# SitaoLuan/When-Do-GNNs-Help

Measured on AMD Instinct MI355X. Metric: aggregation edges/sec (whole job; + %HBM roofline of the SpMM kernel), higher is better.
Workload: dtype f32; 1 GPU; synthetic homophily sweep (data_synthesis/4000-equivalent): 10 h-levels x 5 seeds = 50 graphs/GPU/step, N=2000 nodes, k=10, F=500 fp32, C=5; step = batched D^-1(A+I)X aggregation + edge/label stati...; parallelism=independent sweep shards x1 (no data-path collective; job-table broadcast + r...

## Files before the change

when-do-gnns-help_amd/csrc/spmm_narrow.hip:

```cpp
#include <algorithm>

#include "wdg_common.h"

namespace {
using namespace wdg;

constexpr int N_THREADS = 256;
constexpr int N_WAVES = N_THREADS / kWave;

typedef unsigned short bf16_t;

template <typename TIN>
__device__ __forceinline__ float n_f32(TIN v);
template <>
__device__ __forceinline__ float n_f32<float>(float v) { return v; }
template <>
__device__ __forceinline__ float n_f32<bf16_t>(bf16_t v) { return __uint_as_float(static_cast<unsigned>(v) << 16); }

template <typename TIN>
__global__ __launch_bounds__(256) void narrow_pack(const TIN *__restrict__ X, int64_t ldx, const float *__restrict__ cs, int n_cols,
                                                   int F, float *__restrict__ T) {
    const int64_t i = static_cast<int64_t>(blockIdx.x) * 256 + threadIdx.x;
    if (i >= static_cast<int64_t>(n_cols) * 8) return;
    const int c = static_cast<int>(i >> 3), f = static_cast<int>(i & 7);
    float v = 0.f;
    if (f < F) v = n_f32<TIN>(X[static_cast<int64_t>(c) * ldx + f]) * (cs ? cs[c] : 1.f);
    T[i] = v;
}

template <typename TIN>
__global__ __launch_bounds__(256) void narrow_pack4(const TIN *__restrict__ X, int64_t ldx, const float *__restrict__ cs, int n_cols,
                                                    int F, float *__restrict__ T) {
    const int64_t i = static_cast<int64_t>(blockIdx.x) * 256 + threadIdx.x;
    if (i >= static_cast<int64_t>(n_cols) * 4) return;
    const int c = static_cast<int>(i >> 2), f = static_cast<int>(i & 3);
    float v = 0.f;
    if (f < F) v = n_f32<TIN>(X[static_cast<int64_t>(c) * ldx + f]) * (cs ? cs[c] : 1.f);
    T[i] = v;
}
__global__ __launch_bounds__(256) void narrow_pack_bf16x8(const bf16_t *__restrict__ X, int64_t ldx, int n_cols, int F,
                                                          bf16_t *__restrict__ T) {
    const int64_t i = static_cast<int64_t>(blockIdx.x) * 256 + threadIdx.x;
    if (i >= static_cast<int64_t>(n_cols) * 8) return;
    const int c = static_cast<int>(i >> 3), f = static_cast<int>(i & 7);
    T[i] = f < F ? X[static_cast<int64_t>(c) * ldx + f] : static_cast<bf16_t>(0);
}

enum { TABLE_F32X8 = 0, TABLE_F32X4 = 1, TABLE_BF16X8 = 2 };

struct Acc8 {
    float v[8];
};

__device__ __forceinline__ void narrow_unpack_bf16(const f32x4_t raw, f32x4_t &lo, f32x4_t &hi) {
    const unsigned w0 = __float_as_uint(raw[0]), w1 = __float_as_uint(raw[1]), w2 = __float_as_uint(raw[2]), w3 = __float_as_uint(raw[3]);
    lo[0] = __uint_as_float(w0 << 16); lo[1] = __uint_as_float(w0 & 0xffff0000u);
    lo[2] = __uint_as_float(w1 << 16); lo[3] = __uint_as_float(w1 & 0xffff0000u);
    hi[0] = __uint_as_float(w2 << 16); hi[1] = __uint_as_float(w2 & 0xffff0000u);
    hi[2] = __uint_as_float(w3 << 16); hi[3] = __uint_as_float(w3 & 0xffff0000u);
}

template <int G, bool HAS_W, bool WIDE = true, bool BF16 = false>
__device__ __forceinline__ Acc8 narrow_sweep(global_ptr<const int32_t> col, global_ptr<const float> val,
                                             global_ptr<const f32x4_t> T, int b, int e, int sub, int64_t ldq = 2,
                                             global_ptr<const float> cs = nullptr) {
    Acc8 a;
#pragma unroll
    for (int f = 0; f < 8; ++f) a.v[f] = 0.f;
    const f32x4_t zero = {0.f, 0.f, 0.f, 0.f};
    int k = b + sub;
    for (; k + 3 * G < e; k += 4 * G) {
        int idx[4];
        float w[4];
        f32x4_t lo[4], hi[4];
#pragma unroll
        for (int u = 0; u < 4; ++u) idx[u] = col[k + u * G];
#pragma unroll
        for (int u = 0; u < 4; ++u) {
            lo[u] = T[ldq * static_cast<int64_t>(idx[u])];
            hi[u] = (WIDE && !BF16) ? T[ldq * static_cast<int64_t>(idx[u]) + 1] : zero;
            w[u] = 1.f;
            if (HAS_W) w[u] = (val ? val[k + u * G] : 1.f) * (cs ? cs[idx[u]] : 1.f);
        }
#pragma unroll
        for (int u = 0; u < 4; ++u) {
            if (BF16) narrow_unpack_bf16(lo[u], lo[u], hi[u]);
#pragma unroll
            for (int f = 0; f < 4; ++f) {
                a.v[f] = HAS_W ? __builtin_fmaf(w[u], lo[u][f], a.v[f]) : a.v[f] + lo[u][f];
                if (WIDE) a.v[4 + f] = HAS_W ? __builtin_fmaf(w[u], hi[u][f], a.v[4 + f]) : a.v[4 + f] + hi[u][f];
            }
        }
    }
    for (; k < e; k += G) {
        const int idx = col[k];
        f32x4_t lo = T[ldq * static_cast<int64_t>(idx)], hi = (WIDE && !BF16) ? T[ldq * static_cast<int64_t>(idx) + 1] : zero;
        if (BF16) narrow_unpack_bf16(lo, lo, hi);
        float w = 1.f;
        if (HAS_W) w = (val ? val[k] : 1.f) * (cs ? cs[idx] : 1.f);
#pragma unroll
        for (int f = 0; f < 4; ++f) {
            a.v[f] = HAS_W ? __builtin_fmaf(w, lo[f], a.v[f]) : a.v[f] + lo[f];
            if (WIDE) a.v[4 + f] = HAS_W ? __builtin_fmaf(w, hi[f], a.v[4 + f]) : a.v[4 + f] + hi[f];
        }
    }
    return a;
}

__device__ __forceinline__ float narrow_reduce16(const Acc8 &a, int lane) {
    float h4[4], h2[2];
    const bool b3 = lane & 8, b2 = lane & 4, b1 = lane & 2;
#pragma unroll
    for (int i = 0; i < 4; ++i) {
        const float keep = b3 ? a.v[4 + i] : a.v[i], send = b3 ? a.v[i] : a.v[4 + i];
        h4[i] = keep + __shfl_xor(send, 8);
    }
#pragma unroll
    for (int i = 0; i < 2; ++i) {
        const float keep = b2 ? h4[2 + i] : h4[i], send = b2 ? h4[i] : h4[2 + i];
        h2[i] = keep + __shfl_xor(send, 4);
    }
    const float keep = b1 ? h2[1] : h2[0], send = b1 ? h2[0] : h2[1];
    const float h1 = keep + __shfl_xor(send, 2);
    return h1 + __shfl_xor(h1, 1);
}

__device__ __forceinline__ float narrow_reduce64(Acc8 a, int lane) {
#pragma unroll
    for (int f = 0; f < 8; ++f) a.v[f] += __shfl_xor(a.v[f], 32);
#pragma unroll
    for (int f = 0; f < 8; ++f) a.v[f] += __shfl_xor(a.v[f], 16);
    return narrow_reduce16(a, lane);
}

template <bool HAS_VAL, int TABLE = TABLE_F32X8>
__global__ __launch_bounds__(N_THREADS) void spmm_narrow_kernel(const wdg_spmm_job job, const float *__restrict__ Tf,
                                                                const int32_t *__restrict__ part_ptr, int parts,
                                                                float *__restrict__ P) {
    __shared__ float part_sums[N_WAVES][8];
    constexpr bool WIDE = TABLE != TABLE_F32X4, BF16 = TABLE == TABLE_BF16X8;
    constexpr int64_t LDQ = TABLE == TABLE_F32X8 ? 2 : 1;
    const global_ptr<const int32_t> rowptr = to_global(job.rowptr), col = to_global(job.col), perm = to_global(job.band_perm);
    const global_ptr<const int32_t> pptr = to_global(part_ptr);
    const global_ptr<const float> val = to_global(job.val), rs = to_global(job.row_scale);
    const global_ptr<const f32x4_t> T = (global_ptr<const f32x4_t>)Tf;
    const int N = job.n_rows, F = job.n_feat;
    const int n_wg_rows = job.band_cuts[18], n_wave_rows = job.band_cuts[19];
    const int tid = threadIdx.x, wave = tid >> 6, lane = tid & 63;
    const int feat = (lane >> 1) & 7;
    const int xcd = blockIdx.x % kXcds, per_part = kXcds / parts;
    const int part = xcd / per_part;
    const int wg = (xcd % per_part) + per_part * (blockIdx.x / kXcds), n_wgs = gridDim.x / parts;
    const bool direct = parts == 1;
    const global_ptr<float> out = direct ? to_global(job.Y) : to_global(P) + static_cast<int64_t>(part) * N * 8;
    const int64_t ldo = direct ? job.ldy : 8;
    const int n_out = direct ? F : 8;
    auto bounds = [&](int row, int &b, int &e) {
        b = rowptr[row], e = rowptr[row + 1];
        if (!direct) {
            const global_ptr<const int32_t> pp = pptr + static_cast<int64_t>(row) * (parts - 1);
            if (part > 0) b = pp[part - 1];
            if (part + 1 < parts) e = pp[part];
        }
    };
    auto scale_of = [&](int row) { return (direct && rs) ? rs[row] : 1.f; };

    for (int i = wg; i < n_wg_rows; i += n_wgs) {
        const int row = perm[i];
        int b, e;
        bounds(row, b, e);
        const float total = narrow_reduce64(narrow_sweep<N_THREADS, HAS_VAL, WIDE, BF16>(col, val, T, b, e, tid, LDQ), lane);
        if (lane < 16 && !(lane & 1)) part_sums[wave][feat] = total;
        __syncthreads();
        if (tid < n_out) {
            float sum = part_sums[0][tid];
#pragma unroll
            for (int w = 1; w < N_WAVES; ++w) sum += part_sums[w][tid];
            out[static_cast<int64_t>(row) * ldo + tid] = sum * scale_of(row);
        }
        __syncthreads();
    }
    const int gwave = wg * N_WAVES + wave, n_gwaves = n_wgs * N_WAVES;
    for (int i = n_wg_rows + gwave; i < n_wave_rows; i += n_gwaves) {
        const int row = perm[i];
        int b, e;
        bounds(row, b, e);
        const float total = narrow_reduce64(narrow_sweep<kWave, HAS_VAL, WIDE, BF16>(col, val, T, b, e, lane, LDQ), lane);
        if (lane < 16 && !(lane & 1) && feat < n_out) out[static_cast<int64_t>(row) * ldo + feat] = total * scale_of(row);
    }
    const int rest = N - n_wave_rows;
    for (int q = gwave; q * 4 < rest; q += n_gwaves) {
        const int slot = q * 4 + (lane >> 4);
        const bool live = slot < rest;
        const int row = live ? perm[n_wave_rows + slot] : 0;
        int b = 0, e = 0;
        if (live) bounds(row, b, e);
        const float total = narrow_reduce16(narrow_sweep<16, HAS_VAL, WIDE, BF16>(col, val, T, b, e, lane & 15, LDQ), lane);
        if (live && !(lane & 1) && feat < n_out) out[static_cast<int64_t>(row) * ldo + feat] = total * scale_of(row);
    }
}

__global__ __launch_bounds__(256) void narrow_plan_kernel(const int32_t *__restrict__ rowptr, const int32_t *__restrict__ col, int N,
                                                          int part_cols, int parts, int32_t *__restrict__ part_ptr) {
    const int64_t i = static_cast<int64_t>(blockIdx.x) * 256 + threadIdx.x;
    if (i >= static_cast<int64_t>(N) * (parts - 1)) return;
    const int row = static_cast<int>(i / (parts - 1)), p = static_cast<int>(i % (parts - 1)) + 1;
    int lo = rowptr[row], hi = rowptr[row + 1];
    const int key = p * part_cols;
    while (lo < hi) {
        const int mid = (lo + hi) >> 1;
        if (col[mid] < key) lo = mid + 1;
        else hi = mid;
    }
    part_ptr[i] = lo;
}

__global__ __launch_bounds__(256) void narrow_combine(const float *__restrict__ P, int N, int parts, int F, const float *__restrict__ rs,
                                                      float *__restrict__ Y, int64_t ldy) {
    const int64_t i = static_cast<int64_t>(blockIdx.x) * 256 + threadIdx.x;
    if (i >= static_cast<int64_t>(N) * 8) return;
    const int row = static_cast<int>(i >> 3), f = static_cast<int>(i & 7);
    if (f >= F) return;
    float sum = P[i];
    for (int p = 1; p < parts; ++p) sum += P[static_cast<int64_t>(p) * N * 8 + i];
    Y[static_cast<int64_t>(row) * ldy + f] = sum * (rs ? rs[row] : 1.f);
}

template <bool HAS_W, bool WIDE>
__global__ __launch_bounds__(N_THREADS) void spmm_narrow_batched_kernel(const wdg_spmm_job *__restrict__ jobs, int blocks_per_job) {
    const int job_id = blockIdx.x / blocks_per_job, rb = blockIdx.x % blocks_per_job;
    const desc_ptr<wdg_spmm_job> job = (desc_ptr<wdg_spmm_job>)(jobs + job_id);
    const int N = job->n_rows, F = job->n_feat;
    const int lane = threadIdx.x & 63;
    const int row = rb * 16 + (threadIdx.x >> 4);
    if (rb * 16 >= N) return;
    const global_ptr<const int32_t> rowptr = to_global(job->rowptr), col = to_global(job->col);
    const global_ptr<const float> val = to_global(job->val), rs = to_global(job->row_scale), cs = to_global(job->col_scale);
    const global_ptr<const f32x4_t> X = (global_ptr<const f32x4_t>)to_global(static_cast<const float *>(job->X));
    const bool live = row < N;
    const int b = live ? rowptr[row] : 0, e = live ? rowptr[row + 1] : 0;
    const float total = narrow_reduce16(narrow_sweep<16, HAS_W, WIDE>(col, val, X, b, e, lane & 15, job->ldx / 4, cs), lane);
    const int feat = (lane >> 1) & 7;
    if (live && !(lane & 1) && feat < F) to_global(job->Y)[static_cast<int64_t>(row) * job->ldy + feat] = total * (rs ? rs[row] : 1.f);
}

constexpr int64_t N_PART_BYTES = 3 << 20;

}

extern "C" {

int32_t wdg_spmm_narrow_col_bytes(int32_t n_feat, int32_t x_is_bf16, int32_t has_col_scale) {
    return (n_feat <= 4 || (x_is_bf16 && !has_col_scale)) ? 16 : 32;
}

int32_t wdg_spmm_narrow_parts(int32_t n_cols, int32_t col_bytes) {
    if (const char *s = getenv("WDG_NARROW_PARTS")) {
        const int v = atoi(s);
        if (v == 1 || v == 2 || v == 4 || v == 8) return v;
    }
    int parts = 1;
    while (parts < 8 && static_cast<int64_t>(n_cols) * col_bytes > N_PART_BYTES * parts) parts <<= 1;
    return parts;
}

size_t wdg_spmm_narrow_workspace_bytes(int32_t n_rows, int32_t n_cols) {
    const int parts = wdg_spmm_narrow_parts(n_cols, 32);
    return static_cast<size_t>(n_cols > 0 ? n_cols : 0) * 32 + (parts > 1 ? static_cast<size_t>(parts) * (n_rows > 0 ? n_rows : 0) * 32 : 0) + 512;
}

int wdg_spmm_narrow_plan(const int32_t *rowptr, const int32_t *col, int32_t N, int32_t n_cols, int32_t parts, int32_t *part_ptr,
                         wdg_stream_t stream) {
    WDG_REQUIRE(N >= 0 && n_cols >= 0, "spmm_narrow_plan: negative size");
    WDG_REQUIRE(parts == 1 || parts == 2 || parts == 4 || parts == 8, "spmm_narrow_plan: parts must be 1, 2, 4 or 8");
    if (parts == 1 || N == 0) return WDG_OK;
    WDG_REQUIRE(rowptr && col && part_ptr, "spmm_narrow_plan: null array");
    const int part_cols = static_cast<int>(wdg::ceil_div(n_cols, parts));
    const int64_t threads = static_cast<int64_t>(N) * (parts - 1);
    hipLaunchKernelGGL(narrow_plan_kernel, dim3(static_cast<unsigned>(wdg::ceil_div(threads, 256))), dim3(256), 0, wdg::as_stream(stream),
                       rowptr, col, N, part_cols, parts, part_ptr);
    return wdg::check_launch("narrow_plan_kernel");
}

static int narrow_launch(const wdg_spmm_job *j, bool bf16, const int32_t *part_ptr, void *workspace, size_t workspace_bytes,
                         wdg_stream_t stream) {
    WDG_REQUIRE(j != nullptr, "spmm_narrow: null job");
    WDG_REQUIRE(j->n_rows >= 0 && j->n_cols >= 0 && j->n_feat >= 0, "spmm_narrow: negative size");
    if (j->n_rows == 0 || j->n_feat == 0) return WDG_OK;
    if (j->n_feat > 8) return wdg::fail(WDG_ERR_UNSUPPORTED, "spmm_narrow: more than 8 features (use wdg_spmm_csr_*)");
    WDG_REQUIRE(j->rowptr && j->Y && (j->n_cols == 0 || j->X), "spmm_narrow: null rowptr / X / Y");
    WDG_REQUIRE(j->band_perm && j->band_cuts, "spmm_narrow: the job carries no band plan (wdg_csr_band_plan)");
    WDG_REQUIRE(j->ldx >= j->n_feat && j->ldy >= j->n_feat, "spmm_narrow: leading dimension smaller than n_feat");
    WDG_REQUIRE(j->y_group_stride == 0, "spmm_narrow: Y must be row-major (y_group_stride is the quad-row kernel's)");
    const int col_bytes = wdg_spmm_narrow_col_bytes(j->n_feat, bf16 ? 1 : 0, j->col_scale ? 1 : 0);
    const int table = col_bytes == 32 ? TABLE_F32X8 : (j->n_feat <= 4 ? TABLE_F32X4 : TABLE_BF16X8);
    const int parts = wdg_spmm_narrow_parts(j->n_cols, col_bytes);
    WDG_REQUIRE(parts == 1 || part_ptr, "spmm_narrow: this column count needs the split positions of wdg_spmm_narrow_plan");
    if (!workspace || workspace_bytes < wdg_spmm_narrow_workspace_bytes(j->n_rows, j->n_cols))
        return wdg::fail(WDG_ERR_WORKSPACE, "spmm_narrow: workspace too small");
    hipStream_t st = wdg::as_stream(stream);
    float *T = reinterpret_cast<float *>((reinterpret_cast<uintptr_t>(workspace) + 255) & ~static_cast<uintptr_t>(255));
    float *P = T + static_cast<size_t>(j->n_cols) * 8;
    if (j->n_cols > 0) {
        const int per_col = table == TABLE_F32X4 ? 4 : 8;
        const unsigned blocks = static_cast<unsigned>(wdg::ceil_div(static_cast<int64_t>(j->n_cols) * per_col, 256));
        if (table == TABLE_BF16X8)
            hipLaunchKernelGGL(narrow_pack_bf16x8, dim3(blocks), dim3(256), 0, st, static_cast<const bf16_t *>(j->X), j->ldx, j->n_cols, j->n_feat, reinterpret_cast<bf16_t *>(T));
        else if (table == TABLE_F32X4 && bf16)
            hipLaunchKernelGGL(narrow_pack4<bf16_t>, dim3(blocks), dim3(256), 0, st, static_cast<const bf16_t *>(j->X), j->ldx, j->col_scale, j->n_cols, j->n_feat, T);
        else if (table == TABLE_F32X4)
            hipLaunchKernelGGL(narrow_pack4<float>, dim3(blocks), dim3(256), 0, st, static_cast<const float *>(j->X), j->ldx, j->col_scale, j->n_cols, j->n_feat, T);
        else if (bf16)
            hipLaunchKernelGGL(narrow_pack<bf16_t>, dim3(blocks), dim3(256), 0, st, static_cast<const bf16_t *>(j->X), j->ldx, j->col_scale, j->n_cols, j->n_feat, T);
        else
            hipLaunchKernelGGL(narrow_pack<float>, dim3(blocks), dim3(256), 0, st, static_cast<const float *>(j->X), j->ldx, j->col_scale, j->n_cols, j->n_feat, T);
    }
    const int cus = std::max(wdg_device_cus(), 8);
    const int per_cu = 8;
    const dim3 grid(static_cast<unsigned>(cus / kXcds * kXcds * per_cu));
#define WDG_NARROW_LAUNCH(V, TB) hipLaunchKernelGGL((spmm_narrow_kernel<V, TB>), grid, dim3(N_THREADS), 0, st, *j, T, part_ptr, parts, P)
    if (j->val) {
        if (table == TABLE_F32X8) WDG_NARROW_LAUNCH(true, TABLE_F32X8);
        else if (table == TABLE_F32X4) WDG_NARROW_LAUNCH(true, TABLE_F32X4);
        else WDG_NARROW_LAUNCH(true, TABLE_BF16X8);
    } else {
        if (table == TABLE_F32X8) WDG_NARROW_LAUNCH(false, TABLE_F32X8);
        else if (table == TABLE_F32X4) WDG_NARROW_LAUNCH(false, TABLE_F32X4);
        else WDG_NARROW_LAUNCH(false, TABLE_BF16X8);
    }
#undef WDG_NARROW_LAUNCH
    if (parts > 1) {
        const unsigned blocks = static_cast<unsigned>(wdg::ceil_div(static_cast<int64_t>(j->n_rows) * 8, 256));
        hipLaunchKernelGGL(narrow_combine, dim3(blocks), dim3(256), 0, st, P, j->n_rows, parts, j->n_feat, j->row_scale, j->Y, j->ldy);
    }
    return wdg::check_launch("spmm_narrow_kernel");
}

int wdg_spmm_narrow_f32(const wdg_spmm_job *job_host, const int32_t *part_ptr, void *workspace, size_t workspace_bytes,
                        wdg_stream_t stream) {
    return narrow_launch(job_host, false, part_ptr, workspace, workspace_bytes, stream);
}
int wdg_spmm_narrow_bf16(const wdg_spmm_job *job_host, const int32_t *part_ptr, void *workspace, size_t workspace_bytes,
                         wdg_stream_t stream) {
    return narrow_launch(job_host, true, part_ptr, workspace, workspace_bytes, stream);
}

int wdg_spmm_narrow_batched_f32(const wdg_spmm_job *jobs_dev, int32_t n_jobs, int32_t max_rows, int32_t max_feat, int flags,
                                wdg_stream_t stream) {
    WDG_REQUIRE(n_jobs >= 0 && max_rows >= 0 && max_feat >= 0, "spmm_narrow_batched: negative size");
    if (n_jobs == 0 || max_rows == 0 || max_feat == 0) return WDG_OK;
    WDG_REQUIRE(jobs_dev != nullptr, "spmm_narrow_batched: null job table");
    if (max_feat > 8) return wdg::fail(WDG_ERR_UNSUPPORTED, "spmm_narrow_batched: more than 8 features");
    const int blocks_per_job = static_cast<int>(wdg::ceil_div(max_rows, 16));
    WDG_REQUIRE(static_cast<int64_t>(blocks_per_job) * n_jobs < (1ll << 31), "spmm_narrow_batched: grid too large");
    const dim3 grid(static_cast<unsigned>(blocks_per_job) * n_jobs);
    hipStream_t st = wdg::as_stream(stream);
    const bool has_w = (flags & (WDG_SPMM_ANY_VAL | WDG_SPMM_ANY_COL_SCALE)) != 0, wide = max_feat > 4;
    if (has_w) {
        if (wide) hipLaunchKernelGGL((spmm_narrow_batched_kernel<true, true>), grid, dim3(N_THREADS), 0, st, jobs_dev, blocks_per_job);
        else hipLaunchKernelGGL((spmm_narrow_batched_kernel<true, false>), grid, dim3(N_THREADS), 0, st, jobs_dev, blocks_per_job);
    } else {
        if (wide) hipLaunchKernelGGL((spmm_narrow_batched_kernel<false, true>), grid, dim3(N_THREADS), 0, st, jobs_dev, blocks_per_job);
        else hipLaunchKernelGGL((spmm_narrow_batched_kernel<false, false>), grid, dim3(N_THREADS), 0, st, jobs_dev, blocks_per_job);
    }
    return wdg::check_launch("spmm_narrow_batched_kernel");
}

}
```

Before: 18.68 billion edges/s.

## Process two rows per half-wave in wide batched narrow SpMM and remap blocks across CUs

For the wide case (5-8 features), each 32-lane group now handles two rows. Each lane loads one f32x4 half of a feature row, and the loop is unrolled four edges deep with all loads issued before accumulation, to raise memory-level parallelism. A new reduction combines the two halves with fewer shuffles. Block indices are also permuted in rounds of 8*n_cus so that consecutive blocks of a job spread across compute units. This adds register pressure and a device-query call at launch.

```diff
diff --git a/when-do-gnns-help_amd/csrc/spmm_narrow.hip b/when-do-gnns-help_amd/csrc/spmm_narrow.hip
--- a/when-do-gnns-help_amd/csrc/spmm_narrow.hip
+++ b/when-do-gnns-help_amd/csrc/spmm_narrow.hip
@@ -226,14 +226,118 @@
     Y[static_cast<int64_t>(row) * ldy + f] = sum * (rs ? rs[row] : 1.f);
 }
 
+struct Acc4 {
+    float v[4];
+};
+
+template <bool HAS_W, int R>
+__device__ __forceinline__ void narrow_sweep_pair(global_ptr<const int32_t> col, global_ptr<const float> val, global_ptr<const f32x4_t> T,
+                                                  const int (&b)[R], const int (&e)[R], int slot, int half, int64_t ldq,
+                                                  global_ptr<const float> cs, Acc4 (&a)[R]) {
+    int k[R];
+    bool more = false;
+#pragma unroll
+    for (int r = 0; r < R; ++r) {
+#pragma unroll
+        for (int f = 0; f < 4; ++f) a[r].v[f] = 0.f;
+        k[r] = b[r] + slot;
+        more |= k[r] < e[r];
+    }
+    while (more) {
+        int idx[R][4];
+        float w[R][4];
+        f32x4_t v[R][4];
+        more = false;
+#pragma unroll
+        for (int r = 0; r < R; ++r)
+#pragma unroll
+            for (int u = 0; u < 4; ++u) {
+                idx[r][u] = 0;
+                if (k[r] + 16 * u < e[r]) idx[r][u] = col[k[r] + 16 * u];
+            }
+#pragma unroll
+        for (int r = 0; r < R; ++r)
+#pragma unroll
+            for (int u = 0; u < 4; ++u) {
+                v[r][u] = f32x4_t{0.f, 0.f, 0.f, 0.f};
+                w[r][u] = 1.f;
+                if (k[r] + 16 * u < e[r]) {
+                    v[r][u] = T[ldq * static_cast<int64_t>(static_cast<uint32_t>(idx[r][u])) + half];
+                    if (HAS_W) w[r][u] = (val ? val[k[r] + 16 * u] : 1.f) * (cs ? cs[idx[r][u]] : 1.f);
+                }
+            }
+#pragma unroll
+        for (int r = 0; r < R; ++r) {
+#pragma unroll
+            for (int u = 0; u < 4; ++u)
+                if (k[r] + 16 * u < e[r]) {
+#pragma unroll
+                    for (int f = 0; f < 4; ++f) a[r].v[f] = HAS_W ? __builtin_fmaf(w[r][u], v[r][u][f], a[r].v[f]) : a[r].v[f] + v[r][u][f];
+                }
+            k[r] += 64;
+            more |= k[r] < e[r];
+        }
+    }
+}
+
+__device__ __forceinline__ float narrow_reduce16_pair(const Acc4 &a, int lane) {
+    float h2[2];
+    const bool s3 = lane & 16, s2 = lane & 8;
+#pragma unroll
+    for (int i = 0; i < 2; ++i) {
+        const float keep = s3 ? a.v[2 + i] : a.v[i], send = s3 ? a.v[i] : a.v[2 + i];
+        h2[i] = keep + __shfl_xor(send, 16);
+    }
+    const float keep = s2 ? h2[1] : h2[0], send = s2 ? h2[0] : h2[1];
+    float h1 = keep + __shfl_xor(send, 8);
+    h1 += __shfl_xor(h1, 4);
+    return h1 + __shfl_xor(h1, 2);
+}
+
+template <bool HAS_W>
+__device__ __forceinline__ void narrow_batched_pair(desc_ptr<wdg_spmm_job> job, int rb) {
+    constexpr int R = 2;
+    const int N = job->n_rows, F = job->n_feat;
+    const global_ptr<const int32_t> rowptr = to_global(job->rowptr), col = to_global(job->col);
+    const global_ptr<const float> val = to_global(job->val), rs = to_global(job->row_scale), cs = to_global(job->col_scale);
+    const global_ptr<const f32x4_t> X = (global_ptr<const f32x4_t>)to_global(static_cast<const float *>(job->X));
+    const global_ptr<float> Y = to_global(job->Y);
+    const int64_t ldq = job->ldx / 4, ldy = job->ldy;
+    const int lane = threadIdx.x & 31, slot = lane >> 1, half = lane & 1;
+    const int feat = 4 * half + (slot >> 2);
+    const int row0 = rb * 16 + R * static_cast<int>(threadIdx.x >> 5);
+    int b[R], e[R];
+    float scale[R];
+#pragma unroll
+    for (int r = 0; r < R; ++r) {
+        const int row = row0 + r;
+        b[r] = row < N ? rowptr[row] : 0, e[r] = row < N ? rowptr[row + 1] : 0;
+        scale[r] = (row < N && rs) ? rs[row] : 1.f;
+    }
+    Acc4 a[R];
+    narrow_sweep_pair<HAS_W, R>(col, val, X, b, e, slot, half, ldq, cs, a);
+#pragma unroll
+    for (int r = 0; r < R; ++r) {
+        const int row = row0 + r;
+        const float total = narrow_reduce16_pair(a[r], lane);
+        if (row < N && !(slot & 3) && feat < F) Y[static_cast<int64_t>(row) * ldy + feat] = total * scale[r];
+    }
+}
+
 template <bool HAS_W, bool WIDE>
-__global__ __launch_bounds__(N_THREADS) void spmm_narrow_batched_kernel(const wdg_spmm_job *__restrict__ jobs, int blocks_per_job) {
-    const int job_id = blockIdx.x / blocks_per_job, rb = blockIdx.x % blocks_per_job;
+__global__ __launch_bounds__(N_THREADS) void spmm_narrow_batched_kernel(const wdg_spmm_job *__restrict__ jobs, int blocks_per_job, int n_cus) {
+    const int bid = blockIdx.x, round_size = 8 * n_cus, round = bid / round_size, in = bid % round_size;
+    const int item = (round + 1) * round_size <= static_cast<int>(gridDim.x) ? round * round_size + (in % n_cus) * 8 + in / n_cus : bid;
+    const int job_id = item / blocks_per_job, rb = item % blocks_per_job;
     const desc_ptr<wdg_spmm_job> job = (desc_ptr<wdg_spmm_job>)(jobs + job_id);
     const int N = job->n_rows, F = job->n_feat;
+    if (rb * 16 >= N) return;
+    if constexpr (WIDE) {
+        narrow_batched_pair<HAS_W>(job, rb);
+        return;
+    }
     const int lane = threadIdx.x & 63;
     const int row = rb * 16 + (threadIdx.x >> 4);
-    if (rb * 16 >= N) return;
     const global_ptr<const int32_t> rowptr = to_global(job->rowptr), col = to_global(job->col);
     const global_ptr<const float> val = to_global(job->val), rs = to_global(job->row_scale), cs = to_global(job->col_scale);
     const global_ptr<const f32x4_t> X = (global_ptr<const f32x4_t>)to_global(static_cast<const float *>(job->X));
@@ -354,14 +458,15 @@
     const int blocks_per_job = static_cast<int>(wdg::ceil_div(max_rows, 16));
     WDG_REQUIRE(static_cast<int64_t>(blocks_per_job) * n_jobs < (1ll << 31), "spmm_narrow_batched: grid too large");
     const dim3 grid(static_cast<unsigned>(blocks_per_job) * n_jobs);
+    const int n_cus = std::max(wdg_device_cus(), 8);
     hipStream_t st = wdg::as_stream(stream);
     const bool has_w = (flags & (WDG_SPMM_ANY_VAL | WDG_SPMM_ANY_COL_SCALE)) != 0, wide = max_feat > 4;
     if (has_w) {
-        if (wide) hipLaunchKernelGGL((spmm_narrow_batched_kernel<true, true>), grid, dim3(N_THREADS), 0, st, jobs_dev, blocks_per_job);
-        else hipLaunchKernelGGL((spmm_narrow_batched_kernel<true, false>), grid, dim3(N_THREADS), 0, st, jobs_dev, blocks_per_job);
+        if (wide) hipLaunchKernelGGL((spmm_narrow_batched_kernel<true, true>), grid, dim3(N_THREADS), 0, st, jobs_dev, blocks_per_job, n_cus);
+        else hipLaunchKernelGGL((spmm_narrow_batched_kernel<true, false>), grid, dim3(N_THREADS), 0, st, jobs_dev, blocks_per_job, n_cus);
     } else {
-        if (wide) hipLaunchKernelGGL((spmm_narrow_batched_kernel<false, true>), grid, dim3(N_THREADS), 0, st, jobs_dev, blocks_per_job);
-        else hipLaunchKernelGGL((spmm_narrow_batched_kernel<false, false>), grid, dim3(N_THREADS), 0, st, jobs_dev, blocks_per_job);
+        if (wide) hipLaunchKernelGGL((spmm_narrow_batched_kernel<false, true>), grid, dim3(N_THREADS), 0, st, jobs_dev, blocks_per_job, n_cus);
+        else hipLaunchKernelGGL((spmm_narrow_batched_kernel<false, false>), grid, dim3(N_THREADS), 0, st, jobs_dev, blocks_per_job, n_cus);
     }
     return wdg::check_launch("spmm_narrow_batched_kernel");
 }
```

Result: slower. 18.12 billion edges/s (-3.0%).
